# SGI-2022/Latent-Diffusion-Models-for-Shape-SDFs

Hardware: AMD Instinct MI355X
Metric: SDF queries/sec on 256^3 grid (+ DDPM sample steps/sec) (higher is better)
Workload: dtype bf16; 1 GPU; config4: decode B=64 shapes on a 256^3 grid on 1 rank (the whole grid is the one slab: no gather); batch=64, grid=256, latent_dim=256, decoder=DeepSDF 8x512 skip@4, parallelism=zslab1

## Files before the change

latent-diffusion-models-for-shape-sdfs_amd/csrc/decoder_common.h:

```cpp
#pragma once
#include "grid_index.h"
#include "ldm_internal.h"

#include <math.h>

namespace ldm {
namespace dec {

enum DecMode { kModeGrid = 0, kModePoints = 1, kModeBricks = 2 };

#define LDM_STR2(x) #x
#define LDM_STR(x) LDM_STR2(x)

__device__ __forceinline__ float grid_axis(int i, float vs, float origin) {
#pragma clang fp contract(off)
    float t = (float)i * vs;
    return t + origin;
}

__device__ __forceinline__ void grid_point(int p, int N, int k0, float vs, float origin,
                                           float& x, float& y, float& z) {
    const int nn = N * N;
    const int k = k0 + p / nn;
    const int r = p - (p / nn) * nn;
    const int j = r / N;
    const int i = r - j * N;
    x = grid_axis(i, vs, origin);
    y = grid_axis(j, vs, origin);
    z = grid_axis(k, vs, origin);
}


template <typename T>
struct Elem;
template <>
struct Elem<__bf16> {
    static __device__ __forceinline__ unsigned pack(float a, float b) {
        typedef float f32x2 __attribute__((ext_vector_type(2)));
        const f32x2 v = {a, b};
        return __builtin_bit_cast(unsigned, __builtin_convertvector(v, bf16x2));
    }
    static __device__ __forceinline__ float round(float x) { return (float)(__bf16)x; }
    static __device__ __forceinline__ f32x16 mfma(u32x4 a, u32x4 b, f32x16 c) {
        return __builtin_amdgcn_mfma_f32_32x32x16_bf16(__builtin_bit_cast(bf16x8, a),
                                                       __builtin_bit_cast(bf16x8, b), c, 0, 0, 0);
    }
    static __device__ __forceinline__ f32x16 mfma_v(u32x4 a, u32x4 b) {
        f32x16 d;
        asm volatile("v_mfma_f32_32x32x16_bf16 %0, %1, %2, 0" : "=&v"(d) : "v"(a), "v"(b));
        return d;
    }
    static __device__ __forceinline__ f32x4 mfma16(u32x4 a, u32x4 b, f32x4 c) {
        return __builtin_amdgcn_mfma_f32_16x16x32_bf16(__builtin_bit_cast(bf16x8, a),
                                                       __builtin_bit_cast(bf16x8, b), c, 0, 0, 0);
    }
};
template <>
struct Elem<_Float16> {
    static __device__ __forceinline__ unsigned pack(float a, float b) {
        f16x2 v = {(_Float16)a, (_Float16)b};
        return __builtin_bit_cast(unsigned, v);
    }
    static __device__ __forceinline__ float round(float x) { return (float)(_Float16)x; }
    static __device__ __forceinline__ f32x16 mfma(u32x4 a, u32x4 b, f32x16 c) {
        return __builtin_amdgcn_mfma_f32_32x32x16_f16(__builtin_bit_cast(f16x8, a),
                                                      __builtin_bit_cast(f16x8, b), c, 0, 0, 0);
    }
    static __device__ __forceinline__ f32x16 mfma_v(u32x4 a, u32x4 b) {
        f32x16 d;
        asm volatile("v_mfma_f32_32x32x16_f16 %0, %1, %2, 0" : "=&v"(d) : "v"(a), "v"(b));
        return d;
    }
    static __device__ __forceinline__ f32x4 mfma16(u32x4 a, u32x4 b, f32x4 c) {
        return __builtin_amdgcn_mfma_f32_16x16x32_f16(__builtin_bit_cast(f16x8, a),
                                                      __builtin_bit_cast(f16x8, b), c, 0, 0, 0);
    }
};


__device__ __forceinline__ unsigned relu2(unsigned v) {
    typedef short s16x2 __attribute__((ext_vector_type(2)));
    s16x2 x = __builtin_bit_cast(s16x2, v);
    const s16x2 z = {0, 0};
    x = __builtin_elementwise_max(x, z);
    return __builtin_bit_cast(unsigned, x);
}

template <typename T>
__device__ __forceinline__ void acc_to_frags(const f32x16& a, u32x4& f0, u32x4& f1) {
#pragma unroll
    for (int q = 0; q < 4; ++q) {
        f0[q] = relu2(Elem<T>::pack(a[2 * q], a[2 * q + 1]));
        f1[q] = relu2(Elem<T>::pack(a[8 + 2 * q], a[8 + 2 * q + 1]));
    }
}

}
}
```

latent-diffusion-models-for-shape-sdfs_amd/csrc/decoder_fs.hip:

```cpp
#include "decoder_common.h"

namespace ldm {
namespace {
using namespace dec;

constexpr int kFsD = 4;

constexpr int kFsStep = 2048;
constexpr int kFsAct = 33 * 4 * 1024;
constexpr int kFsRed = 4 * 4 * 64 * 4;
constexpr int kFsWl = 512 * 4;
#ifndef FS_STAMP
#define FS_STAMP 0
#endif
constexpr int kFsStamp = FS_STAMP ? 128 * 8 : 0;
#ifndef FS_ABL
#define FS_ABL 0
#endif
static_assert(FS_ABL == 0 || FS_STAMP, "ablations are diagnostic builds");
constexpr int kFsLds = kFsAct + kFsRed + kFsWl + kFsStamp;
static_assert(kFsLds <= 160 * 1024, "LDS");

__host__ __device__ constexpr int fs_nparts(int S) { return S == 256 ? 15 : 16; }
__host__ __device__ constexpr int fs_nsteps(int S) { return S == 256 ? 384 : 448; }

template <typename T>
__global__ void fs_aux_pack_kernel(const float* __restrict__ beta, const float* __restrict__ wxyz,
                                   int B, T* __restrict__ aux) {
    const int id = blockIdx.x * blockDim.x + threadIdx.x;
    if (id >= B * 4 * 4 * 2 * 64) return;
    const int lane = id & 63;
    const int i = (id >> 6) & 1;
    const int slot = (id >> 7) & 3;
    const int w = (id >> 9) & 3;
    const int b = id >> 11;
    const int li = slot >> 1;
    const int p = slot & 1;
    float v[8] = {0, 0, 0, 0, 0, 0, 0, 0};
    if (lane < 32) {
        const int f = 128 * w + 64 * p + 32 * i + lane;
        const float* wx = wxyz + ((size_t)li * kHidden + f) * 3;
        const float bb = beta[((size_t)b * 2 + li) * kHidden + f];
        const float hi = Elem<T>::round(bb);
        v[0] = wx[0]; v[1] = wx[1]; v[2] = wx[2];
        v[3] = wx[0]; v[4] = wx[1]; v[5] = wx[2];
        v[6] = hi;    v[7] = bb - hi;
    }
    T* o = aux + (size_t)id * 8;
#pragma unroll
    for (int e = 0; e < 8; ++e) o[e] = (T)v[e];
}

struct FArgs {
    const uint8_t* stream;
    const uint8_t* aux;
    const float* w_last;
    const float* xyz;
    float* out;
    float b_last;
    int npts, tiles_per_shape, n_tiles;
    int N, k0;
    float vs, origin;
    const int32_t* bricks;
    const int32_t* count;
    int nb, nbt;
    GridDiv gd;
};

enum FsEpi { FE_NONE = 0, FE_LATE = 1, FE_EARLY = 2, FE_FIN0 = 3, FE_FIN1 = 4, FE_CVT = 5,
             FE_WR = 6, FE_PIN = 8 };

struct FSrc {
    bool shape;
    uint32_t off;
    bool none = false;
};

struct FCtx {
    int lane, wave, h;
    uint32_t voff;
    char* smem;
    __amdgpu_buffer_rsrc_t rw;
    __amdgpu_buffer_rsrc_t ra;
    uint32_t s_beg, s_end;
    uint32_t s_iss;
    uint32_t baux_w;
    uint32_t aux_w;
    uint32_t aux_next;
    u32x4 auxn[2];
    u32x4 ring[kFsD][2];
    u32x4 b[4];
    float part[4];
    u32x4 ef[16];
    float* out;
    int npts, prev_shape, prev_local;
    float b_last;
    unsigned long long* st;
    int st_i;
    bool st_on;
    const int32_t* bricks;
    int N, nb, nbt;
};

__device__ __forceinline__ void stamp(FCtx& c) {
    if (FS_STAMP) {
        if (c.st_on && c.lane == 0 && c.st_i < 128) c.st[c.st_i] = __builtin_readcyclecounter();
        ++c.st_i;
    }
}

__device__ __forceinline__ u32x4 bld(__amdgpu_buffer_rsrc_t r, uint32_t voff, uint32_t soff) {
    return __builtin_bit_cast(u32x4, __builtin_amdgcn_raw_buffer_load_b128(r, voff, soff, 0));
}

__device__ __forceinline__ void load_aux(FCtx& c, FSrc s) {
    if (s.none) return;
    const __amdgpu_buffer_rsrc_t r = s.shape ? c.ra : c.rw;
    c.auxn[0] = bld(r, c.voff, s.off);
    c.auxn[1] = bld(r, c.voff + 1024u, s.off);
}

__device__ __forceinline__ uint32_t opaque(uint32_t v) {
    asm volatile("" : "+v"(v));
    return v;
}

__device__ __forceinline__ int opaque_s(int v) {
    asm volatile("" : "+s"(v));
    return v;
}

__device__ __forceinline__ char* lds_at(const FCtx& c, uint32_t off) {
    return c.smem + (opaque(c.voff) + off);
}
__device__ __forceinline__ u32x4* act_w(const FCtx& c, int late) {
    return reinterpret_cast<u32x4*>(lds_at(c, (uint32_t)(late + 4 * c.wave) * 4096u));
}
__device__ __forceinline__ const f32x4* wl_at(const FCtx& c, int p, int i) {
    const uint32_t h = opaque(c.voff) >> 9;
    return reinterpret_cast<const f32x4*>(
        c.smem + kFsAct + kFsRed + (((c.wave * 2 + p) * 2 + i) * 2) * 64 + h * 64);
}

__device__ __forceinline__ float* red_w(const FCtx& c) {
    return reinterpret_cast<float*>(c.smem + kFsAct + c.wave * 4 * 64 * 4 + (opaque(c.voff) >> 2));
}

__device__ __forceinline__ void fs_bar() {
    if (FS_ABL & 4) return;
    asm volatile("s_waitcnt lgkmcnt(0)\n\ts_barrier" ::: "memory");
}

__device__ __forceinline__ void read_b(FCtx& c, int pos) {
    const u32x4* p = reinterpret_cast<const u32x4*>(lds_at(c, pos * 4096));
#pragma unroll
    for (int n = 0; n < 4; ++n) c.b[n] = p[n * 64];
}

__device__ __forceinline__ void issue(FCtx& c, int r) {
    const uint32_t so = c.s_iss + (uint32_t)(r >> 1) * 2u * kFsStep;
    const uint32_t vo = c.voff + (uint32_t)(r & 1) * kFsStep;
    if (FS_ABL & 1) return;
    c.ring[r][0] = bld(c.rw, vo, so);
    c.ring[r][1] = bld(c.rw, vo + 1024u, so);
}

__device__ __forceinline__ void next_group(FCtx& c) {
    c.s_iss += 4u * kFsStep;
    if (c.s_iss == c.s_end) c.s_iss = c.s_beg;
}

__device__ __forceinline__ float relu_f(float x) {
    return __builtin_bit_cast(float, max(__builtin_bit_cast(int, x), 0));
}

__device__ __forceinline__ float acc_read(float a) {
    asm volatile("" : "+a"(a));
    return a;
}

template <typename T, int EKP>
__device__ __forceinline__ void epi_unit(FCtx& c, const f32x16 (&accY)[2][4], int u,
                                         u32x4* wbase) {
    constexpr int EK = EKP & 7;
    constexpr bool PIN = (EKP & FE_PIN) != 0 || EK == FE_FIN1;
    const int t = u >> 1, s = u & 1;
    const int i = t >> 2, n = t & 3;
    if (FS_ABL & 2) return;
    if (EK == FE_LATE || EK == FE_EARLY) {
        u32x4 f;
#pragma unroll
        for (int q = 0; q < 4; ++q) {
            const float lo = accY[i][n][8 * s + 2 * q], hi = accY[i][n][8 * s + 2 * q + 1];
            f[q] = relu2(PIN ? Elem<T>::pack(acc_read(lo), acc_read(hi)) : Elem<T>::pack(lo, hi));
        }
        wbase[((2 * i + s) * 4 + n) * 64] = f;
    } else if (EK == FE_FIN0 || EK == FE_FIN1) {
        const f32x4* w = wl_at(c, EK == FE_FIN0 ? 0 : 1, i);
        float part = c.part[n];
#pragma unroll
        for (int q = 2 * s; q < 2 * s + 2; ++q) {
            const f32x4 wv = w[q];
#pragma unroll
            for (int e = 0; e < 4; ++e) {
                const float v = PIN ? acc_read(accY[i][n][4 * q + e]) : accY[i][n][4 * q + e];
                part = fmaf(relu_f(v), wv[e], part);
            }
        }
        c.part[n] = part;
    }
}

template <typename T, int EKP>
__device__ __forceinline__ void epi_step(FCtx& c, const f32x16 (&accY)[2][4], int k,
                                         u32x4* wbase) {
    constexpr int EK = EKP & 7;
    if (EK == FE_NONE || k == 15) return;
    if (EK == FE_CVT) {
        if ((FS_ABL & 2) || k >= 8) return;
        u32x4 f0, f1;
#pragma unroll
        for (int q = 0; q < 4; ++q) {
            const f32x16& a = accY[k >> 2][k & 3];
            f0[q] = relu2(Elem<T>::pack(acc_read(a[2 * q]), acc_read(a[2 * q + 1])));
            f1[q] = relu2(Elem<T>::pack(acc_read(a[8 + 2 * q]), acc_read(a[8 + 2 * q + 1])));
        }
        c.ef[2 * k] = f0;
        c.ef[2 * k + 1] = f1;
        return;
    }
    if (EK == FE_WR) {
        if ((FS_ABL & 2) || k >= 4) return;
#pragma unroll
        for (int t = 2 * k; t < 2 * k + 2; ++t) {
            const int i = t >> 2, n = t & 3;
            wbase[(2 * i * 4 + n) * 64] = c.ef[2 * t];
            wbase[((2 * i + 1) * 4 + n) * 64] = c.ef[2 * t + 1];
        }
        return;
    }
    epi_unit<T, EKP>(c, accY, k, wbase);
    if (k == 14) epi_unit<T, EKP>(c, accY, 15, wbase);
    if (EK == FE_FIN0 && k == 14) {
#pragma unroll
        for (int n = 0; n < 4; ++n) asm volatile("" : "+v"(c.part[n]));
    }
    if (EK == FE_FIN1 && k == 14) {
        float* rw = red_w(c);
#pragma unroll
        for (int n = 0; n < 4; ++n) {
            rw[n * 64] = c.part[n];
            c.part[n] = 0.f;
        }
    }
}

__device__ __forceinline__ void fin_store(const FCtx& c, int shape, int local) {
    const int lane = (int)(opaque(c.voff) >> 4);
    if (local < 0 || lane >= 32) return;
    const float* rr = reinterpret_cast<const float*>(
        c.smem + kFsAct + c.wave * 64 * 4 + (opaque(c.voff) >> 2));
    float s = 0.f;
#pragma unroll
    for (int w = 0; w < 4; ++w) s += rr[w * 4 * 64] + rr[w * 4 * 64 + 32];
    const int pt = local * kTilePoints + 32 * c.wave + lane;
    if (pt < c.npts) {
        const __amdgpu_buffer_rsrc_t ro = __builtin_amdgcn_make_buffer_rsrc(
            (void*)(c.out + (size_t)shape * c.npts), (short)0, 0x7ffffff0, 0x00020000);
        __builtin_amdgcn_raw_buffer_store_b32(__builtin_bit_cast(uint32_t, tanhf(s + c.b_last)),
                                              ro, (uint32_t)pt * 4u, 0, 2 );
    }
}

__device__ __forceinline__ int list_at(const int32_t* list, int i) {
    typedef const __attribute__((address_space(4))) int32_t* const_i32;
    return ((const_i32)(uintptr_t)list)[i];
}

__device__ __forceinline__ void brick_origin(int gid, int nb_, int& shape, int& i0, int& j0,
                                             int& k0) {
    const int nb = opaque_s(nb_);
    const int nb2 = nb * nb, nb3 = nb2 * nb;
    shape = gid / nb3;
    const int id = gid - shape * nb3;
    const int bz = id / nb2, r = id - bz * nb2;
    const int by = r / nb;
    i0 = 8 * (r - by * nb);
    j0 = 8 * by;
    k0 = 8 * bz;
}

__device__ __forceinline__ void fin_store_bricks(const FCtx& c, int tile) {
    const int lane = (int)(opaque(c.voff) >> 4);
    if (tile < 0 || lane >= 32) return;
    const float* rr = reinterpret_cast<const float*>(
        c.smem + kFsAct + c.wave * 64 * 4 + (opaque(c.voff) >> 2));
    float s = 0.f;
#pragma unroll
    for (int w = 0; w < 4; ++w) s += rr[w * 4 * 64] + rr[w * 4 * 64 + 32];
    const int gid = list_at(c.bricks, tile >> 2);
    LDM_DASSERT(gid >= 0 && gid < c.nbt);
    int shape, i0, j0, k0;
    brick_origin(gid, c.nb, shape, i0, j0, k0);
    const int idx = 128 * (tile & 3) + 32 * c.wave + lane;
    const int i = i0 + (idx & 7), j = j0 + ((idx >> 3) & 7);
    const int k = k0 + 2 * (tile & 3) + (c.wave >> 1);
    const int N = c.N;
    if ((unsigned)gid < (unsigned)c.nbt && i < N && j < N && k < N) {
        const __amdgpu_buffer_rsrc_t ro = __builtin_amdgcn_make_buffer_rsrc(
            (void*)(c.out + ((size_t)shape * N + k) * N * N), (short)0, 0x7ffffff0, 0x00020000);
        __builtin_amdgcn_raw_buffer_store_b32(__builtin_bit_cast(uint32_t, tanhf(s + c.b_last)),
                                              ro, (uint32_t)(j * N + i) * 4u, 0, 2 );
    }
}

template <int MODE>
__device__ __forceinline__ void fin_store_mode(const FCtx& c) {
    if (MODE == kModeBricks) fin_store_bricks(c, c.prev_local);
    else fin_store(c, c.prev_shape, c.prev_local);
}

__device__ __forceinline__ void valu_slot(int v) {
    if (v == 2) __builtin_amdgcn_sched_group_barrier(0x002, 2, 0);
    else if (v == 4) __builtin_amdgcn_sched_group_barrier(0x002, 4, 0);
}

template <typename T>
__device__ __forceinline__ void mfma_pair(f32x16 (&acc)[2][4], const u32x4& a0, const u32x4& a1,
                                          const u32x4& b, int n) {
    acc[0][n] = Elem<T>::mfma(a0, b, acc[0][n]);
    acc[1][n] = Elem<T>::mfma(a1, b, acc[1][n]);
}

template <typename T, int EKP, int K0, int BAR>
__device__ __forceinline__ void group4(FCtx& c, f32x16 (&acc)[2][4], const f32x16 (&accY)[2][4],
                                       int p0) {
    constexpr int EK = EKP & 7;
    constexpr int BP = 1;
    u32x4* wbase = nullptr;
    if (EK == FE_LATE) wbase = act_w(c, 16);
    if (EK == FE_EARLY || EK == FE_WR) wbase = act_w(c, 0);
    const char* gbase = lds_at(c, (p0 + 1) * 4096);
#pragma unroll
    for (int r = 0; r < 4; ++r) {
        const u32x4* nb = reinterpret_cast<const u32x4*>(gbase + r * 4096);
        const u32x4 a0 = c.ring[r][0], a1 = c.ring[r][1];
        const int k = K0 + r;
        const int V = (EK == FE_NONE || EK == FE_WR || k == 15) ? 0
                      : (k == 14 || EK == FE_CVT) ? 4 : 2;
        if (r == BAR) {
#pragma unroll
            for (int n = 0; n < BP; ++n) mfma_pair<T>(acc, a0, a1, c.b[n], n);
            for (int n = 0; n < BP; ++n) {
                __builtin_amdgcn_sched_group_barrier(0x008, 2, 0);
            }
            __builtin_amdgcn_sched_barrier(0);
            fs_bar();
            __builtin_amdgcn_sched_barrier(0);
#pragma unroll
            for (int n = 0; n < BP; ++n) c.b[n] = nb[n * 64];
#pragma unroll
            for (int n = BP; n < 4; ++n) {
                mfma_pair<T>(acc, a0, a1, c.b[n], n);
                c.b[n] = nb[n * 64];
            }
            issue(c, r);
            epi_step<T, EKP>(c, accY, k, wbase);
            for (int n = 0; n < BP; ++n) __builtin_amdgcn_sched_group_barrier(0x100, 1, 0);
            for (int n = BP; n < 4; ++n) {
                __builtin_amdgcn_sched_group_barrier(0x008, 1, 0);
                valu_slot(V);
                __builtin_amdgcn_sched_group_barrier(0x008, 1, 0);
                __builtin_amdgcn_sched_group_barrier(0x100, 1, 0);
                valu_slot(V);
            }
        } else {
#pragma unroll
            for (int n = 0; n < 4; ++n) {
                mfma_pair<T>(acc, a0, a1, c.b[n], n);
                c.b[n] = nb[n * 64];
            }
            issue(c, r);
            epi_step<T, EKP>(c, accY, k, wbase);
#pragma unroll
            for (int n = 0; n < 4; ++n) {
                __builtin_amdgcn_sched_group_barrier(0x008, 1, 0);
                valu_slot(V);
                __builtin_amdgcn_sched_group_barrier(0x008, 1, 0);
                __builtin_amdgcn_sched_group_barrier(0x100, 1, 0);
                valu_slot(V);
            }
        }
        __builtin_amdgcn_sched_group_barrier(0x020, 2, 0);
        __builtin_amdgcn_sched_barrier(0);
    }
    next_group(c);
}

template <typename T, int EK, bool BAR>
__device__ __forceinline__ void steps16e(FCtx& c, f32x16 (&acc)[2][4],
                                         const f32x16 (&accY)[2][4], int p0) {
    group4<T, EK, 0, -1>(c, acc, accY, p0);
    group4<T, EK, 4, -1>(c, acc, accY, p0 + 4);
    group4<T, EK, 8, -1>(c, acc, accY, p0 + 8);
    group4<T, EK, 12, BAR ? 3 : -1>(c, acc, accY, p0 + 12);
}

template <typename T>
__device__ __forceinline__ void steps_plain(FCtx& c, f32x16 (&acc)[2][4],
                                            const f32x16 (&accY)[2][4], int pos0, int j0, int j1) {
#pragma unroll 1
    for (int j = j0; j < j1; j += 4) group4<T, FE_NONE, 0, -1>(c, acc, accY, pos0 + j);
}

template <typename T, int EKP, bool E16, int MODE = kModeGrid>
__device__ __forceinline__ void run_part(FCtx& c, f32x16 (&acc)[2][4], const f32x16 (&accY)[2][4],
                                         int nk, bool mid, bool endbar, FSrc naux, int pos0,
                                         bool bar0) {
    constexpr int EK = EKP & 7;
    const f32x16 zero = {};
    const u32x4 a0 = c.auxn[0], a1 = c.auxn[1];
    if (bar0) {
#pragma unroll
        for (int n = 0; n < 4; ++n) {
            acc[0][n] = Elem<T>::mfma(a0, c.b[n], zero);
            acc[1][n] = Elem<T>::mfma(a1, c.b[n], zero);
        }
        load_aux(c, naux);
        fs_bar();
        read_b(c, pos0);
    } else {
        const u32x4* p = reinterpret_cast<const u32x4*>(lds_at(c, pos0 * 4096));
#pragma unroll
        for (int n = 0; n < 4; ++n) {
            acc[0][n] = Elem<T>::mfma(a0, c.b[n], zero);
            acc[1][n] = Elem<T>::mfma(a1, c.b[n], zero);
            c.b[n] = p[n * 64];
        }
        load_aux(c, naux);
#pragma unroll
        for (int n = 0; n < 4; ++n) {
            __builtin_amdgcn_sched_group_barrier(0x008, 2, 0);
            __builtin_amdgcn_sched_group_barrier(0x100, 1, 0);
        }
        __builtin_amdgcn_sched_group_barrier(0x020, 2, 0);
        __builtin_amdgcn_sched_barrier(0);
    }
    if (EK == FE_NONE) {
#pragma unroll
        for (int i = 0; i < 2; ++i)
#pragma unroll
            for (int n = 0; n < 4; ++n) asm volatile("" ::"a"(accY[i][n]));
    }
    stamp(c);
    if (!E16 && EK != FE_NONE) {
        if (mid || (endbar && nk == 16)) steps16e<T, EKP, true>(c, acc, accY, pos0);
        else steps16e<T, EKP, false>(c, acc, accY, pos0);
        if (EK == FE_FIN1) {
            stamp(c);
            fin_store_mode<MODE>(c);
        }
        stamp(c);
        if (endbar && nk == 32) {
            steps_plain<T>(c, acc, accY, pos0, 16, 28);
            group4<T, FE_NONE, 0, 3>(c, acc, accY, pos0 + 28);
        } else {
            steps_plain<T>(c, acc, accY, pos0, 16, nk);
        }
    } else if (E16 && (EKP & FE_PIN)) {
        steps_plain<T>(c, acc, accY, pos0, 0, 12);
        group4<T, FE_NONE, 0, 3>(c, acc, accY, pos0 + 12);
        stamp(c);
        if (endbar) steps16e<T, EKP, true>(c, acc, accY, pos0 + 16);
        else steps16e<T, EKP, false>(c, acc, accY, pos0 + 16);
    } else if (E16) {
        static_assert(!E16 || EK == FE_EARLY, "E16 parts convert part 0 of their own layer");
        steps_plain<T>(c, acc, accY, pos0, 0, 8);
        group4<T, FE_CVT, 0, -1>(c, acc, accY, pos0 + 8);
        group4<T, FE_CVT, 4, 3>(c, acc, accY, pos0 + 12);
        stamp(c);
        group4<T, FE_WR, 0, -1>(c, acc, accY, pos0 + 16);
        steps_plain<T>(c, acc, accY, pos0, 20, 28);
        group4<T, FE_NONE, 0, 3>(c, acc, accY, pos0 + 28);
    } else {
        steps_plain<T>(c, acc, accY, pos0, 0, nk < 16 ? nk : 16);
        stamp(c);
        steps_plain<T>(c, acc, accY, pos0, 16, nk);
    }
    stamp(c);
}

template <typename T>
__device__ __forceinline__ void acc_to_lds(FCtx& c, const f32x16 (&acc)[2][4]) {
    u32x4* p = act_w(c, 16);
#pragma unroll
    for (int i = 0; i < 2; ++i)
#pragma unroll
        for (int n = 0; n < 4; ++n) {
            u32x4 f0, f1;
            acc_to_frags<T>(acc[i][n], f0, f1);
            p[(2 * i * 4 + n) * 64] = f0;
            p[((2 * i + 1) * 4 + n) * 64] = f1;
        }
}

template <typename T, bool LATE>
__device__ __forceinline__ void layer0_part(FCtx& c, FSrc naux) {
    const u32x4 a[2] = {c.auxn[0], c.auxn[1]};
    u32x4* p = act_w(c, LATE ? 16 : 0);
    f32x16 t[2];
    t[0] = Elem<T>::mfma_v(a[0], c.b[0]);
#pragma unroll
    for (int q = 0; q < 8; ++q) {
        const int i = q & 1, n = q >> 1;
        if (q < 7) t[(q + 1) & 1] = Elem<T>::mfma_v(a[(q + 1) & 1], c.b[(q + 1) >> 1]);
        if (q == 0) {
            asm volatile("s_nop 10" : "+v"(t[0]));
            load_aux(c, naux);
            stamp(c);
        }
        __builtin_amdgcn_sched_barrier(0);
        u32x4 f0, f1;
        acc_to_frags<T>(t[q & 1], f0, f1);
        p[(2 * i * 4 + n) * 64] = f0;
        p[((2 * i + 1) * 4 + n) * 64] = f1;
        __builtin_amdgcn_sched_barrier(0);
    }
    stamp(c);
}

template <typename T, int S, int MODE>
__global__ __launch_bounds__(256, 1) void dec_fs_kernel(FArgs a) {
    __shared__ __attribute__((aligned(16))) char smem[kFsLds];
    FCtx c;
    c.lane = threadIdx.x & 63;
    c.wave = __builtin_amdgcn_readfirstlane(threadIdx.x >> 6);
// ... 74 lines not shown
        stamp(c);
        load_aux(c, shp(0));
        const uint32_t lv = opaque(c.voff);
        const bool hi = lv >= 512u;
        const uint32_t p0 = (uint32_t)local * kTilePoints;
        uint32_t ti = 0, tj = 0, tk = 0;
        if (MODE == kModeGrid) {
            grid_first(p0, (uint32_t)a.N, a.gd, ti, tj, tk);
            tk += (uint32_t)a.k0;
        }
        const float* row = nullptr;
        if (MODE == kModePoints) {
            row = a.xyz + (size_t)shape * a.npts * 3;
            asm volatile("" : "+s"(row));
        }
#pragma unroll
        for (int n = 0; n < 4; ++n) {
            int pt = local * kTilePoints + 32 * n + (int)((lv >> 4) & 31u);
            if (pt >= a.npts) pt = a.npts - 1;
            float x, y, z;
            if (MODE == kModeBricks) {
                const int idx = 128 * (tile & 3) + 32 * n + (int)((lv >> 4) & 31u);
                const int m = a.N - 1;
                x = grid_axis(min(bi0 + (idx & 7), m), a.vs, a.origin);
                y = grid_axis(min(bj0 + ((idx >> 3) & 7), m), a.vs, a.origin);
                z = grid_axis(min(bk0 + (idx >> 6), m), a.vs, a.origin);
            } else if (MODE == kModePoints) {
                const float* qq = row + (size_t)pt * 3;
                x = qq[0];
                y = qq[1];
                z = qq[2];
            } else {
                const uint32_t off =
                    grid_tail_off(p0, 32u * n + ((lv >> 4) & 31u), (uint32_t)a.npts);
                uint32_t vi, vj, vk;
                grid_voxel(ti, tj, tk, off, (uint32_t)a.N, a.gd.m, vi, vj, vk);
                x = grid_axis((int)vi, a.vs, a.origin);
                y = grid_axis((int)vj, a.vs, a.origin);
                z = grid_axis((int)vk, a.vs, a.origin);
            }
            const float xh = Elem<T>::round(x), yh = Elem<T>::round(y), zh = Elem<T>::round(z);
            u32x4 f;
            f[0] = hi ? 0u : Elem<T>::pack(xh, yh);
            f[1] = hi ? 0u : Elem<T>::pack(zh, x - xh);
            f[2] = hi ? 0u : Elem<T>::pack(y - yh, z - zh);
            f[3] = hi ? 0u : Elem<T>::pack(1.f, 1.f);
            reinterpret_cast<u32x4*>(lds_at(c, 32u * 4096u))[n * 64] = f;
        }
        read_b(c, 32);

        layer0_part<T, false>(c, shp(1));
        layer0_part<T, true>(c, bias(2));

        constexpr int kPinW = S == 512 ? FE_PIN : 0;
        int pi = 2;
        run_part<T, FE_FIN1, false, MODE>(c, accA, accB, 32, true, false, bias(pi + 1), 0, true);
        run_part<T, FE_EARLY, true>(c, accB, accA, 32, true, true, bias(pi + 2), 0, false);
        pi += 2;
        constexpr int L2P = S == 256 ? 3 : 4;
#pragma unroll 1
        for (int l = 2; l < L2P; ++l, pi += 2) {
            const FSrc nx = (S == 512 && l == 3) ? shp(2) : bias(pi + 2);
            run_part<T, FE_LATE | kPinW, false>(c, accA, accB, 32, true, false, bias(pi + 1), 0,
                                                false);
            run_part<T, FE_EARLY | FE_PIN, true>(c, accB, accA, 32, true, true, nx, 0, false);
        }
        if (S == 256) {
            run_part<T, FE_LATE | kPinW, false>(c, accA, accB, 32, true, false, shp(2), 0,
                                                false);
            fs_bar();
            acc_to_lds<T>(c, accA);
            stamp(c);
            run_part<T, FE_NONE, false>(c, accA, accB, 16, false, false, shp(3), 16, true);
            run_part<T, FE_EARLY | FE_PIN, false>(c, accB, accA, 16, false, true, bias(pi + 3),
                                                  16, false);
            pi += 3;
        } else {
            run_part<T, FE_LATE | kPinW, false>(c, accA, accB, 32, true, false, shp(3), 0,
                                                false);
            run_part<T, FE_EARLY | FE_PIN, true>(c, accB, accA, 32, true, true, bias(pi + 2), 0,
                                                 false);
            pi += 2;
        }
#pragma unroll 1
        for (int l = 5; l < 7; ++l, pi += 2) {
            run_part<T, FE_LATE | FE_PIN, false>(c, accA, accB, 32, true, false, bias(pi + 1), 0,
                                                 false);
            run_part<T, FE_EARLY | FE_PIN, true>(c, accB, accA, 32, true, true, bias(pi + 2), 0,
                                                 false);
        }
        run_part<T, FE_LATE | FE_PIN, false>(c, accA, accB, 32, true, false, bias(pi + 1), 0,
                                             false);
        run_part<T, FE_FIN0 | FE_PIN, false>(c, accB, accA, 32, false, true, FSrc{true, 0, true},
                                             0, false);
        c.prev_shape = shape;
        c.prev_local = local;
        c.aux_w = c.aux_next;
    }
#pragma unroll
    for (int u = 0; u < 16; ++u) epi_unit<T, FE_FIN1>(c, accB, u, nullptr);
    {
        float* rw = red_w(c);
#pragma unroll
        for (int n = 0; n < 4; ++n) rw[n * 64] = c.part[n];
    }
    fs_bar();
    fin_store_mode<MODE>(c);
    asm volatile("s_waitcnt vmcnt(0)" ::: "memory");
    if (FS_STAMP && c.wave == 0) {
        __builtin_amdgcn_s_waitcnt(0);
        for (int k = c.lane; k < 128; k += 64)
            reinterpret_cast<unsigned long long*>(a.out)[(size_t)blockIdx.x * 128 + k] = c.st[k];
    }
}

template <typename T, int S>
void launch_fs(const FArgs& a, bool points, hipStream_t s, int grid) {
    if (points)
        hipLaunchKernelGGL((dec_fs_kernel<T, S, kModePoints>), dim3(grid), dim3(256), 0, s, a);
    else
        hipLaunchKernelGGL((dec_fs_kernel<T, S, kModeGrid>), dim3(grid), dim3(256), 0, s, a);
}

template <typename T, int S>
void launch_fs_bricks(const FArgs& a, hipStream_t s, int grid) {
    hipLaunchKernelGGL((dec_fs_kernel<T, S, kModeBricks>), dim3(grid), dim3(256), 0, s, a);
}

}

size_t decoder_fs_aux_bytes(int B) { return (size_t)B * 4 * 4 * kFsStep; }

int decoder_fs_n_stages(int skip_width) { return fs_nsteps(skip_width == 253 ? 256 : 512); }

int decoder_fs_fwd(const ldm_decoder_t* w, const float* beta, const float* xyz, int B, int npts,
                   int N, int k0, float vs, float origin, float* out, void* ws, size_t ws_bytes,
                   hipStream_t s, int num_cus, const int32_t* bricks, const int32_t* count,
                   int n_bricks) {
    const int S = w->skip_width == 253 ? 256 : 512;
    LDM_REQUIRE(w->n_stages == fs_nsteps(S), LDM_EINVAL, "split layout: n_stages %d != %d",
                w->n_stages, fs_nsteps(S));
    LDM_REQUIRE(ws != nullptr && ws_bytes >= decoder_fs_aux_bytes(B) && LDM_ALIGNED(ws, 16),
                LDM_ENOSPC, "workspace too small: need %zu bytes, got %zu",
                decoder_fs_aux_bytes(B), ws_bytes);
    LDM_REQUIRE((size_t)B * 4 * 4 * kFsStep < 0x7ffffff0u, LDM_EINVAL,
                "split layout: %d shapes exceed the aux buffer range", B);
    {
        const int n = B * 4 * 4 * 2 * 64;
        if (w->dtype == LDM_BF16)
            hipLaunchKernelGGL(fs_aux_pack_kernel<__bf16>, dim3((n + 255) / 256), dim3(256), 0, s,
                               beta, w->wxyz, B, (__bf16*)ws);
        else
            hipLaunchKernelGGL(fs_aux_pack_kernel<_Float16>, dim3((n + 255) / 256), dim3(256), 0,
// ... 46 lines not shown
```

Measured before the change: 457.7 million queries/s.

## Interleave accumulator epilogue with MFMA pairs via inline asm windows

Replaces the separate epilogue step (epi_unit/epi_step with FE_PIN/FE_CVT/FE_WR variants) with hand-scheduled inline-asm MFMA pairs. Each pair reads previous-layer accumulators from AGPRs, converts and applies relu, or accumulates the final-layer dot product, in the shadow of the matrix ops. It also precomputes LDS base pointers per 16-step group and carries the stream issue offset across groups, which cuts address arithmetic. The aim is to hide VALU epilogue work behind MFMA latency, but the fixed asm ordering limits what the compiler can schedule and adds register-pressure risk.

```diff
diff --git a/latent-diffusion-models-for-shape-sdfs_amd/csrc/decoder_common.h b/latent-diffusion-models-for-shape-sdfs_amd/csrc/decoder_common.h
--- a/latent-diffusion-models-for-shape-sdfs_amd/csrc/decoder_common.h
+++ b/latent-diffusion-models-for-shape-sdfs_amd/csrc/decoder_common.h
@@ -31,6 +31,120 @@
 }
 
 
+#define LDM_PAIR_OPS(MFMA, CVT)                                                                   \
+                                                                       \
+    template <bool TAIL>                                                                          \
+    static __device__ __forceinline__ void pair_cvt1(f32x16& c0, f32x16& c1, const u32x4& a0,     \
+                                                     const u32x4& a1, const u32x4& b, float e0,   \
+                                                     float e1, unsigned& w) {                     \
+        unsigned t0, t1;                                                                          \
+        if (!TAIL)                                                                                \
+            asm volatile(MFMA " %0, %5, %7, %0\n\t"                                               \
+                         "v_accvgpr_read_b32 %3, %8\n\t"                                          \
+                         "v_accvgpr_read_b32 %4, %9\n\t"                                          \
+                         MFMA " %1, %6, %7, %1\n\t"                                               \
+                         CVT " %2, %3, %4\n\t"                                                    \
+                         "v_pk_max_i16 %2, %2, 0"                                                 \
+                         : "+a"(c0), "+a"(c1), "=&v"(w), "=&v"(t0), "=&v"(t1)                     \
+                         : "v"(a0), "v"(a1), "v"(b), "a"(e0), "a"(e1));                           \
+        else                                                                                      \
+            asm volatile(MFMA " %0, %5, %7, %0\n\t"                                               \
+                         "v_accvgpr_read_b32 %3, %8\n\t"                                          \
+                         "v_accvgpr_read_b32 %4, %9\n\t"                                          \
+                         CVT " %2, %3, %4\n\t"                                                    \
+                         "v_pk_max_i16 %2, %2, 0\n\t"                                             \
+                         MFMA " %1, %6, %7, %1"                                                   \
+                         : "+a"(c0), "+a"(c1), "=&v"(w), "=&v"(t0), "=&v"(t1)                     \
+                         : "v"(a0), "v"(a1), "v"(b), "a"(e0), "a"(e1));                           \
+    }                                                                                             \
+                                                                                  \
+    template <bool TAIL>                                                                          \
+    static __device__ __forceinline__ void pair_cvt2(f32x16& c0, f32x16& c1, const u32x4& a0,     \
+                                                     const u32x4& a1, const u32x4& b, float e0,   \
+                                                     float e1, float e2, float e3, unsigned& w0,  \
+                                                     unsigned& w1) {                              \
+        unsigned t0, t1;                                                                          \
+        if (!TAIL)                                                                                \
+            asm volatile(MFMA " %0, %6, %8, %0\n\t"                                               \
+                         "v_accvgpr_read_b32 %4, %9\n\t"                                          \
+                         "v_accvgpr_read_b32 %5, %10\n\t"                                         \
+                         CVT " %2, %4, %5\n\t"                                                    \
+                         "v_pk_max_i16 %2, %2, 0\n\t"                                             \
+                         MFMA " %1, %7, %8, %1\n\t"                                               \
+                         "v_accvgpr_read_b32 %4, %11\n\t"                                         \
+                         "v_accvgpr_read_b32 %5, %12\n\t"                                         \
+                         CVT " %3, %4, %5\n\t"                                                    \
+                         "v_pk_max_i16 %3, %3, 0"                                                 \
+                         : "+a"(c0), "+a"(c1), "=&v"(w0), "=&v"(w1), "=&v"(t0), "=&v"(t1)         \
+                         : "v"(a0), "v"(a1), "v"(b), "a"(e0), "a"(e1), "a"(e2), "a"(e3));         \
+        else                                                                                      \
+            asm volatile(MFMA " %0, %6, %8, %0\n\t"                                               \
+                         "v_accvgpr_read_b32 %4, %9\n\t"                                          \
+                         "v_accvgpr_read_b32 %5, %10\n\t"                                         \
+                         CVT " %2, %4, %5\n\t"                                                    \
+                         "v_pk_max_i16 %2, %2, 0\n\t"                                             \
+                         "v_accvgpr_read_b32 %4, %11\n\t"                                         \
+                         "v_accvgpr_read_b32 %5, %12\n\t"                                         \
+                         MFMA " %1, %7, %8, %1\n\t"                                               \
+                         CVT " %3, %4, %5\n\t"                                                    \
+                         "v_pk_max_i16 %3, %3, 0"                                                 \
+                         : "+a"(c0), "+a"(c1), "=&v"(w0), "=&v"(w1), "=&v"(t0), "=&v"(t1)         \
+                         : "v"(a0), "v"(a1), "v"(b), "a"(e0), "a"(e1), "a"(e2), "a"(e3));         \
+    }                                                                                             \
+              \
+    template <bool TAIL>                                                                          \
+    static __device__ __forceinline__ void pair_fin(f32x16& c0, f32x16& c1, const u32x4& a0,      \
+                                                    const u32x4& a1, const u32x4& b, float e0,    \
+                                                    float e1, float w0, float w1, float& p) {     \
+        float t0, t1;                                                                             \
+        if (!TAIL)                                                                                \
+            asm volatile(MFMA " %0, %5, %7, %0\n\t"                                               \
+                         "v_accvgpr_read_b32 %3, %8\n\t"                                          \
+                         "v_accvgpr_read_b32 %4, %9\n\t"                                          \
+                         "v_max_i32_e32 %3, 0, %3\n\t"                                            \
+                         "v_max_i32_e32 %4, 0, %4\n\t"                                            \
+                         MFMA " %1, %6, %7, %1\n\t"                                               \
+                         "v_fmac_f32_e32 %2, %3, %10\n\t"                                         \
+                         "v_fmac_f32_e32 %2, %4, %11"                                             \
+                         : "+a"(c0), "+a"(c1), "+v"(p), "=&v"(t0), "=&v"(t1)                      \
+                         : "v"(a0), "v"(a1), "v"(b), "a"(e0), "a"(e1), "v"(w0), "v"(w1));         \
+        else                                                                                      \
+            asm volatile(MFMA " %0, %5, %7, %0\n\t"                                               \
+                         "v_accvgpr_read_b32 %3, %8\n\t"                                          \
+                         "v_accvgpr_read_b32 %4, %9\n\t"                                          \
+                         "v_max_i32_e32 %3, 0, %3\n\t"                                            \
+                         "v_max_i32_e32 %4, 0, %4\n\t"                                            \
+                         "v_fmac_f32_e32 %2, %3, %10\n\t"                                         \
+                         "v_fmac_f32_e32 %2, %4, %11\n\t"                                         \
+                         MFMA " %1, %6, %7, %1"                                                   \
+                         : "+a"(c0), "+a"(c1), "+v"(p), "=&v"(t0), "=&v"(t1)                      \
+                         : "v"(a0), "v"(a1), "v"(b), "a"(e0), "a"(e1), "v"(w0), "v"(w1));         \
+    }                                                                                             \
+                    \
+    static __device__ __forceinline__ void pair_fin3(f32x16& c0, f32x16& c1, const u32x4& a0,     \
+                                                     const u32x4& a1, const u32x4& b, float e0,   \
+                                                     float e1, float w0, float w1, float& p,      \
+                                                     float x, float wx, float& q) {               \
+        float t0, t1, t2;                                                                         \
+        asm volatile(MFMA " %0, %7, %9, %0\n\t"                                                   \
+                     "v_accvgpr_read_b32 %4, %10\n\t"                                             \
+                     "v_accvgpr_read_b32 %5, %11\n\t"                                             \
+                     "v_max_i32_e32 %4, 0, %4\n\t"                                                \
+                     "v_max_i32_e32 %5, 0, %5\n\t"                                                \
+                     "v_accvgpr_read_b32 %6, %12\n\t"                                             \
+                     MFMA " %1, %8, %9, %1\n\t"                                                   \
+                     "v_fmac_f32_e32 %2, %4, %13\n\t"                                             \
+                     "v_fmac_f32_e32 %2, %5, %14\n\t"                                             \
+                     "v_max_i32_e32 %6, 0, %6\n\t"                                                \
+                     "v_fmac_f32_e32 %3, %6, %15"                                                 \
+                     : "+a"(c0), "+a"(c1), "+v"(p), "+v"(q), "=&v"(t0), "=&v"(t1), "=&v"(t2)      \
+                     : "v"(a0), "v"(a1), "v"(b), "a"(e0), "a"(e1), "a"(x), "v"(w0), "v"(w1),      \
+                       "v"(wx));                                                                  \
+    }
+
+#define LDM_CVT_BF16 "v_cvt_pk_bf16_f32"
+#define LDM_CVT_F16 "v_cvt_pk_f16_f32"
+
 template <typename T>
 struct Elem;
 template <>
@@ -54,6 +168,7 @@
         return __builtin_amdgcn_mfma_f32_16x16x32_bf16(__builtin_bit_cast(bf16x8, a),
                                                        __builtin_bit_cast(bf16x8, b), c, 0, 0, 0);
     }
+    LDM_PAIR_OPS("v_mfma_f32_32x32x16_bf16", LDM_CVT_BF16)
 };
 template <>
 struct Elem<_Float16> {
@@ -75,6 +190,7 @@
         return __builtin_amdgcn_mfma_f32_16x16x32_f16(__builtin_bit_cast(f16x8, a),
                                                       __builtin_bit_cast(f16x8, b), c, 0, 0, 0);
     }
+    LDM_PAIR_OPS("v_mfma_f32_32x32x16_f16", LDM_CVT_F16)
 };
 
 
diff --git a/latent-diffusion-models-for-shape-sdfs_amd/csrc/decoder_fs.hip b/latent-diffusion-models-for-shape-sdfs_amd/csrc/decoder_fs.hip
--- a/latent-diffusion-models-for-shape-sdfs_amd/csrc/decoder_fs.hip
+++ b/latent-diffusion-models-for-shape-sdfs_amd/csrc/decoder_fs.hip
@@ -67,8 +67,7 @@
     GridDiv gd;
 };
 
-enum FsEpi { FE_NONE = 0, FE_LATE = 1, FE_EARLY = 2, FE_FIN0 = 3, FE_FIN1 = 4, FE_CVT = 5,
-             FE_WR = 6, FE_PIN = 8 };
+enum FsEpi { FE_NONE = 0, FE_LATE = 1, FE_EARLY = 2, FE_FIN0 = 3, FE_FIN1 = 4 };
 
 struct FSrc {
     bool shape;
@@ -91,7 +90,8 @@
     u32x4 ring[kFsD][2];
     u32x4 b[4];
     float part[4];
-    u32x4 ef[16];
+    const f32x4* wlp;
+    f32x4 wl[2][4];
     float* out;
     int npts, prev_shape, prev_local;
     float b_last;
@@ -133,6 +133,12 @@
 __device__ __forceinline__ char* lds_at(const FCtx& c, uint32_t off) {
     return c.smem + (opaque(c.voff) + off);
 }
+__device__ __forceinline__ char* lds_base(const FCtx& c, uint32_t off) {
+    return c.smem + opaque(opaque(c.voff) + off);
+}
+__device__ __forceinline__ u32x4* act_wb(const FCtx& c, int late) {
+    return reinterpret_cast<u32x4*>(lds_base(c, (uint32_t)(late + 4 * c.wave) * 4096u));
+}
 __device__ __forceinline__ u32x4* act_w(const FCtx& c, int late) {
     return reinterpret_cast<u32x4*>(lds_at(c, (uint32_t)(late + 4 * c.wave) * 4096u));
 }
@@ -165,10 +171,11 @@
     c.ring[r][1] = bld(c.rw, vo + 1024u, so);
 }
 
-__device__ __forceinline__ void next_group(FCtx& c) {
-    c.s_iss += 4u * kFsStep;
-    if (c.s_iss == c.s_end) c.s_iss = c.s_beg;
-}
+__device__ __forceinline__ uint32_t next_iss(const FCtx& c) {
+    const uint32_t n = c.s_iss + 4u * kFsStep;
+    return n == c.s_end ? c.s_beg : n;
+}
+__device__ __forceinline__ void next_group(FCtx& c) { c.s_iss = next_iss(c); }
 
 __device__ __forceinline__ float relu_f(float x) {
     return __builtin_bit_cast(float, max(__builtin_bit_cast(int, x), 0));
@@ -179,80 +186,141 @@
     return a;
 }
 
-template <typename T, int EKP>
-__device__ __forceinline__ void epi_unit(FCtx& c, const f32x16 (&accY)[2][4], int u,
-                                         u32x4* wbase) {
-    constexpr int EK = EKP & 7;
-    constexpr bool PIN = (EKP & FE_PIN) != 0 || EK == FE_FIN1;
+__device__ __forceinline__ void fin1_unit(FCtx& c, const f32x16 (&accY)[2][4], int u) {
     const int t = u >> 1, s = u & 1;
     const int i = t >> 2, n = t & 3;
-    if (FS_ABL & 2) return;
-    if (EK == FE_LATE || EK == FE_EARLY) {
+    const f32x4* w = wl_at(c, 1, i);
+    float part = c.part[n];
+#pragma unroll
+    for (int q = 2 * s; q < 2 * s + 2; ++q) {
+        const f32x4 wv = w[q];
+#pragma unroll
+        for (int e = 0; e < 4; ++e)
+            part = fmaf(relu_f(acc_read(accY[i][n][4 * q + e])), wv[e], part);
+    }
+    c.part[n] = part;
+}
+
+template <typename T>
+__device__ __forceinline__ void mfma_pair(f32x16 (&acc)[2][4], const u32x4& a0, const u32x4& a1,
+                                          const u32x4& b, int n) {
+    acc[0][n] = Elem<T>::mfma(a0, b, acc[0][n]);
+    acc[1][n] = Elem<T>::mfma(a1, b, acc[1][n]);
+}
+
+template <typename T>
+__device__ __forceinline__ void window_step(FCtx& c, f32x16 (&acc)[2][4],
+                                            const f32x16 (&accY)[2][4], const u32x4& a0,
+                                            const u32x4& a1, const u32x4* nb, int k, int r,
+                                            u32x4* wbase) {
+    uint32_t nxt = 0;
+    if (k < 14) {
+        const int t = k >> 1, s = k & 1;
+        const int i = t >> 2, nn = t & 3;
         u32x4 f;
 #pragma unroll
-        for (int q = 0; q < 4; ++q) {
-            const float lo = accY[i][n][8 * s + 2 * q], hi = accY[i][n][8 * s + 2 * q + 1];
-            f[q] = relu2(PIN ? Elem<T>::pack(acc_read(lo), acc_read(hi)) : Elem<T>::pack(lo, hi));
-        }
-        wbase[((2 * i + s) * 4 + n) * 64] = f;
-    } else if (EK == FE_FIN0 || EK == FE_FIN1) {
-        const f32x4* w = wl_at(c, EK == FE_FIN0 ? 0 : 1, i);
-        float part = c.part[n];
-#pragma unroll
-        for (int q = 2 * s; q < 2 * s + 2; ++q) {
-            const f32x4 wv = w[q];
-#pragma unroll
-            for (int e = 0; e < 4; ++e) {
-                const float v = PIN ? acc_read(accY[i][n][4 * q + e]) : accY[i][n][4 * q + e];
-                part = fmaf(relu_f(v), wv[e], part);
+        for (int n = 0; n < 4; ++n) {
+            unsigned w;
+            if (r == 3 && n == 1) nxt = next_iss(c);
+            const float e0 = accY[i][nn][8 * s + 2 * n], e1 = accY[i][nn][8 * s + 2 * n + 1];
+            if (n < 3)
+                Elem<T>::template pair_cvt1<false>(acc[0][n], acc[1][n], a0, a1, c.b[n], e0, e1,
+                                                   w);
+            else
+                Elem<T>::template pair_cvt1<true>(acc[0][n], acc[1][n], a0, a1, c.b[n], e0, e1,
+                                                  w);
+            f[n] = w;
+            c.b[n] = nb[n * 64];
+            __builtin_amdgcn_sched_barrier(0);
+        }
+        issue(c, r);
+        wbase[((2 * i + s) * 4 + nn) * 64] = f;
+        if (r == 3) c.s_iss = nxt;
+    } else {
+        u32x4 f[2];
+        const f32x16& y = accY[1][3];
+#pragma unroll
+        for (int p = 0; p < 4; ++p) {
+            unsigned w0, w1;
+            if (p < 3)
+                Elem<T>::template pair_cvt2<false>(acc[0][p], acc[1][p], a0, a1, c.b[p], y[4 * p],
+                                                   y[4 * p + 1], y[4 * p + 2], y[4 * p + 3], w0,
+                                                   w1);
+            else
+                Elem<T>::template pair_cvt2<true>(acc[0][p], acc[1][p], a0, a1, c.b[p], y[4 * p],
+                                                  y[4 * p + 1], y[4 * p + 2], y[4 * p + 3], w0,
+                                                  w1);
+            f[p >> 1][2 * (p & 1)] = w0;
+            f[p >> 1][2 * (p & 1) + 1] = w1;
+            c.b[p] = nb[p * 64];
+            if (p == 1) wbase[(2 * 4 + 3) * 64] = f[0];
+            __builtin_amdgcn_sched_barrier(0);
+        }
+        issue(c, r);
+        wbase[(3 * 4 + 3) * 64] = f[1];
+    }
+    __builtin_amdgcn_sched_barrier(0);
+}
+
+template <typename T, int P>
+__device__ __forceinline__ void window_step_fin(FCtx& c, f32x16 (&acc)[2][4],
+                                                const f32x16 (&accY)[2][4], const u32x4& a0,
+                                                const u32x4& a1, const u32x4* nb, int k, int r) {
+    const int t = k >> 1, s = k & 1;
+    const int i = t >> 2, nn = t & 3;
+    const f32x16& y = accY[1][3];
+    uint32_t nxt = 0;
+    if (k == 0) {
+        c.wlp = wl_at(c, P, 0);
+#pragma unroll
+        for (int q = 0; q < 4; ++q) c.wl[0][q] = c.wlp[q];
+    }
+#pragma unroll
+    for (int n = 0; n < 4; ++n) {
+        if (k < 14) {
+            const int e = 8 * s + 2 * n;
+            const float e0 = accY[i][nn][e], e1 = accY[i][nn][e + 1];
+            const float w0 = c.wl[i][e >> 2][e & 3], w1 = c.wl[i][e >> 2][(e & 3) + 1];
+            const int x = 2 * (k - 8) + n;
+            if (k >= 8 && n < 2)
+                Elem<T>::pair_fin3(acc[0][n], acc[1][n], a0, a1, c.b[n], e0, e1, w0, w1,
+                                   c.part[nn], y[x], c.wl[1][x >> 2][x & 3], c.part[3]);
+            else if (n < 3)
+                Elem<T>::template pair_fin<false>(acc[0][n], acc[1][n], a0, a1, c.b[n], e0, e1,
+                                                  w0, w1, c.part[nn]);
+            else
+                Elem<T>::template pair_fin<true>(acc[0][n], acc[1][n], a0, a1, c.b[n], e0, e1,
+                                                 w0, w1, c.part[nn]);
+        } else if (n < 2) {
+            const int x = 12 + 2 * n;
+            Elem<T>::template pair_fin<false>(acc[0][n], acc[1][n], a0, a1, c.b[n], y[x],
+                                              y[x + 1], c.wl[1][3][x & 3],
+                                              c.wl[1][3][(x & 3) + 1],
+                                              c.part[3]);
+        } else {
+            mfma_pair<T>(acc, a0, a1, c.b[n], n);
+        }
+        if (r == 3 && n == 2) nxt = next_iss(c);
+        c.b[n] = nb[n * 64];
+        if (k == 6) c.wl[1][n] = c.wlp[8 + n];
+        if (k == 14 && n == 2) {
+            if (P == 0) {
+#pragma unroll
+                for (int m = 0; m < 4; ++m) asm volatile("" : "+v"(c.part[m]));
+            } else {
+                float* rw = red_w(c);
+#pragma unroll
+                for (int m = 0; m < 4; ++m) {
+                    rw[m * 64] = c.part[m];
+                    c.part[m] = 0.f;
+                }
             }
         }
-        c.part[n] = part;
-    }
-}
-
-template <typename T, int EKP>
-__device__ __forceinline__ void epi_step(FCtx& c, const f32x16 (&accY)[2][4], int k,
-                                         u32x4* wbase) {
-    constexpr int EK = EKP & 7;
-    if (EK == FE_NONE || k == 15) return;
-    if (EK == FE_CVT) {
-        if ((FS_ABL & 2) || k >= 8) return;
-        u32x4 f0, f1;
-#pragma unroll
-        for (int q = 0; q < 4; ++q) {
-            const f32x16& a = accY[k >> 2][k & 3];
-            f0[q] = relu2(Elem<T>::pack(acc_read(a[2 * q]), acc_read(a[2 * q + 1])));
-            f1[q] = relu2(Elem<T>::pack(acc_read(a[8 + 2 * q]), acc_read(a[8 + 2 * q + 1])));
-        }
-        c.ef[2 * k] = f0;
-        c.ef[2 * k + 1] = f1;
-        return;
-    }
-    if (EK == FE_WR) {
-        if ((FS_ABL & 2) || k >= 4) return;
-#pragma unroll
-        for (int t = 2 * k; t < 2 * k + 2; ++t) {
-            const int i = t >> 2, n = t & 3;
-            wbase[(2 * i * 4 + n) * 64] = c.ef[2 * t];
-            wbase[((2 * i + 1) * 4 + n) * 64] = c.ef[2 * t + 1];
-        }
-        return;
-    }
-    epi_unit<T, EKP>(c, accY, k, wbase);
-    if (k == 14) epi_unit<T, EKP>(c, accY, 15, wbase);
-    if (EK == FE_FIN0 && k == 14) {
-#pragma unroll
-        for (int n = 0; n < 4; ++n) asm volatile("" : "+v"(c.part[n]));
-    }
-    if (EK == FE_FIN1 && k == 14) {
-        float* rw = red_w(c);
-#pragma unroll
-        for (int n = 0; n < 4; ++n) {
-            rw[n * 64] = c.part[n];
-            c.part[n] = 0.f;
-        }
-    }
+        __builtin_amdgcn_sched_barrier(0);
+    }
+    issue(c, r);
+    if (r == 3) c.s_iss = nxt;
+    __builtin_amdgcn_sched_barrier(0);
 }
 
 __device__ __forceinline__ void fin_store(const FCtx& c, int shape, int local) {
@@ -320,34 +388,26 @@
     else fin_store(c, c.prev_shape, c.prev_local);
 }
 
-__device__ __forceinline__ void valu_slot(int v) {
-    if (v == 2) __builtin_amdgcn_sched_group_barrier(0x002, 2, 0);
-    else if (v == 4) __builtin_amdgcn_sched_group_barrier(0x002, 4, 0);
-}
-
-template <typename T>
-__device__ __forceinline__ void mfma_pair(f32x16 (&acc)[2][4], const u32x4& a0, const u32x4& a1,
-                                          const u32x4& b, int n) {
-    acc[0][n] = Elem<T>::mfma(a0, b, acc[0][n]);
-    acc[1][n] = Elem<T>::mfma(a1, b, acc[1][n]);
-}
-
-template <typename T, int EKP, int K0, int BAR>
+template <typename T, int EK, int K0, int BAR, bool WIN = false>
 __device__ __forceinline__ void group4(FCtx& c, f32x16 (&acc)[2][4], const f32x16 (&accY)[2][4],
-                                       int p0) {
-    constexpr int EK = EKP & 7;
+                                       int p0, const char* gb = nullptr, u32x4* wb = nullptr,
+                                       uint32_t* go = nullptr) {
+    static_assert(WIN || EK == FE_NONE, "windows run through steps16e");
     constexpr int BP = 1;
-    u32x4* wbase = nullptr;
-    if (EK == FE_LATE) wbase = act_w(c, 16);
-    if (EK == FE_EARLY || EK == FE_WR) wbase = act_w(c, 0);
-    const char* gbase = lds_at(c, (p0 + 1) * 4096);
+    const bool carry = go != nullptr;
+    const char* gbase = WIN ? gb : carry ? c.smem + *go + 4096 : lds_base(c, (p0 + 1) * 4096);
 #pragma unroll
     for (int r = 0; r < 4; ++r) {
-        const u32x4* nb = reinterpret_cast<const u32x4*>(gbase + r * 4096);
+        const bool last = carry && r == 3;
+        uint32_t nxt = 0;
+        if (last) {
+            nxt = next_iss(c);
+            *go = opaque(*go + 4u * 4096u);
+        }
+        const u32x4* nb =
+            reinterpret_cast<const u32x4*>(last ? c.smem + *go : gbase + r * 4096);
         const u32x4 a0 = c.ring[r][0], a1 = c.ring[r][1];
         const int k = K0 + r;
-        const int V = (EK == FE_NONE || EK == FE_WR || k == 15) ? 0
-                      : (k == 14 || EK == FE_CVT) ? 4 : 2;
         if (r == BAR) {
 #pragma unroll
             for (int n = 0; n < BP; ++n) mfma_pair<T>(acc, a0, a1, c.b[n], n);
@@ -365,15 +425,19 @@
                 c.b[n] = nb[n * 64];
             }
             issue(c, r);
-            epi_step<T, EKP>(c, accY, k, wbase);
             for (int n = 0; n < BP; ++n) __builtin_amdgcn_sched_group_barrier(0x100, 1, 0);
             for (int n = BP; n < 4; ++n) {
-                __builtin_amdgcn_sched_group_barrier(0x008, 1, 0);
-                valu_slot(V);
-                __builtin_amdgcn_sched_group_barrier(0x008, 1, 0);
+                __builtin_amdgcn_sched_group_barrier(0x008, 2, 0);
                 __builtin_amdgcn_sched_group_barrier(0x100, 1, 0);
-                valu_slot(V);
             }
+        } else if ((EK == FE_LATE || EK == FE_EARLY) && k < 15 && !(FS_ABL & 2)) {
+            window_step<T>(c, acc, accY, a0, a1, nb, k, r, wb);
+            if (r == 3) return;
+            continue;
+        } else if ((EK == FE_FIN0 || EK == FE_FIN1) && k < 15 && !(FS_ABL & 2)) {
+            window_step_fin<T, EK == FE_FIN1>(c, acc, accY, a0, a1, nb, k, r);
+            if (r == 3) return;
+            continue;
         } else {
 #pragma unroll
             for (int n = 0; n < 4; ++n) {
@@ -381,43 +445,48 @@
                 c.b[n] = nb[n * 64];
             }
             issue(c, r);
-            epi_step<T, EKP>(c, accY, k, wbase);
+            if (last) c.s_iss = nxt;
 #pragma unroll
             for (int n = 0; n < 4; ++n) {
-                __builtin_amdgcn_sched_group_barrier(0x008, 1, 0);
-                valu_slot(V);
-                __builtin_amdgcn_sched_group_barrier(0x008, 1, 0);
+                __builtin_amdgcn_sched_group_barrier(0x008, 2, 0);
+                if (last && n == 0) {
+                    __builtin_amdgcn_sched_group_barrier(0x004, 3, 0);
+                    __builtin_amdgcn_sched_group_barrier(0x002, 1, 0);
+                }
                 __builtin_amdgcn_sched_group_barrier(0x100, 1, 0);
-                valu_slot(V);
             }
         }
         __builtin_amdgcn_sched_group_barrier(0x020, 2, 0);
         __builtin_amdgcn_sched_barrier(0);
     }
-    next_group(c);
+    if (!carry) next_group(c);
 }
 
 template <typename T, int EK, bool BAR>
 __device__ __forceinline__ void steps16e(FCtx& c, f32x16 (&acc)[2][4],
                                          const f32x16 (&accY)[2][4], int p0) {
-    group4<T, EK, 0, -1>(c, acc, accY, p0);
-    group4<T, EK, 4, -1>(c, acc, accY, p0 + 4);
-    group4<T, EK, 8, -1>(c, acc, accY, p0 + 8);
-    group4<T, EK, 12, BAR ? 3 : -1>(c, acc, accY, p0 + 12);
+    const char* gb = lds_base(c, (p0 + 1) * 4096);
+    u32x4* wb = EK == FE_LATE ? act_wb(c, 16) : EK == FE_EARLY ? act_wb(c, 0) : nullptr;
+    group4<T, EK, 0, -1, true>(c, acc, accY, p0, gb, wb);
+    group4<T, EK, 4, -1, true>(c, acc, accY, p0 + 4, gb + 4 * 4096, wb);
+    group4<T, EK, 8, -1, true>(c, acc, accY, p0 + 8, gb + 8 * 4096, wb);
+    group4<T, EK, 12, BAR ? 3 : -1, true>(c, acc, accY, p0 + 12, gb + 12 * 4096, wb);
 }
 
 template <typename T>
 __device__ __forceinline__ void steps_plain(FCtx& c, f32x16 (&acc)[2][4],
                                             const f32x16 (&accY)[2][4], int pos0, int j0, int j1) {
+    if (j0 >= j1) return;
+    uint32_t go = opaque(opaque(c.voff) + (uint32_t)(pos0 + j0) * 4096u);
 #pragma unroll 1
-    for (int j = j0; j < j1; j += 4) group4<T, FE_NONE, 0, -1>(c, acc, accY, pos0 + j);
-}
-
-template <typename T, int EKP, bool E16, int MODE = kModeGrid>
+    for (int j = j0; j < j1; j += 4)
+        group4<T, FE_NONE, 0, -1>(c, acc, accY, pos0 + j, nullptr, nullptr, &go);
+}
+
+template <typename T, int EK, bool E16, int MODE = kModeGrid>
 __device__ __forceinline__ void run_part(FCtx& c, f32x16 (&acc)[2][4], const f32x16 (&accY)[2][4],
                                          int nk, bool mid, bool endbar, FSrc naux, int pos0,
                                          bool bar0) {
-    constexpr int EK = EKP & 7;
     const f32x16 zero = {};
     const u32x4 a0 = c.auxn[0], a1 = c.auxn[1];
     if (bar0) {
@@ -454,8 +523,8 @@
     }
     stamp(c);
     if (!E16 && EK != FE_NONE) {
-        if (mid || (endbar && nk == 16)) steps16e<T, EKP, true>(c, acc, accY, pos0);
-        else steps16e<T, EKP, false>(c, acc, accY, pos0);
+        if (mid || (endbar && nk == 16)) steps16e<T, EK, true>(c, acc, accY, pos0);
+        else steps16e<T, EK, false>(c, acc, accY, pos0);
         if (EK == FE_FIN1) {
             stamp(c);
             fin_store_mode<MODE>(c);
@@ -467,21 +536,13 @@
         } else {
             steps_plain<T>(c, acc, accY, pos0, 16, nk);
         }
-    } else if (E16 && (EKP & FE_PIN)) {
+    } else if (E16) {
+        static_assert(!E16 || EK == FE_EARLY, "E16 parts convert part 0 of their own layer");
         steps_plain<T>(c, acc, accY, pos0, 0, 12);
         group4<T, FE_NONE, 0, 3>(c, acc, accY, pos0 + 12);
         stamp(c);
-        if (endbar) steps16e<T, EKP, true>(c, acc, accY, pos0 + 16);
-        else steps16e<T, EKP, false>(c, acc, accY, pos0 + 16);
-    } else if (E16) {
-        static_assert(!E16 || EK == FE_EARLY, "E16 parts convert part 0 of their own layer");
-        steps_plain<T>(c, acc, accY, pos0, 0, 8);
-        group4<T, FE_CVT, 0, -1>(c, acc, accY, pos0 + 8);
-        group4<T, FE_CVT, 4, 3>(c, acc, accY, pos0 + 12);
-        stamp(c);
-        group4<T, FE_WR, 0, -1>(c, acc, accY, pos0 + 16);
-        steps_plain<T>(c, acc, accY, pos0, 20, 28);
-        group4<T, FE_NONE, 0, 3>(c, acc, accY, pos0 + 28);
+        if (endbar) steps16e<T, EK, true>(c, acc, accY, pos0 + 16);
+        else steps16e<T, EK, false>(c, acc, accY, pos0 + 16);
     } else {
         steps_plain<T>(c, acc, accY, pos0, 0, nk < 16 ? nk : 16);
         stamp(c);
@@ -662,7 +723,6 @@
         layer0_part<T, false>(c, shp(1));
         layer0_part<T, true>(c, bias(2));
 
-        constexpr int kPinW = S == 512 ? FE_PIN : 0;
         int pi = 2;
         run_part<T, FE_FIN1, false, MODE>(c, accA, accB, 32, true, false, bias(pi + 1), 0, true);
         run_part<T, FE_EARLY, true>(c, accB, accA, 32, true, true, bias(pi + 2), 0, false);
@@ -671,44 +731,44 @@
 #pragma unroll 1
         for (int l = 2; l < L2P; ++l, pi += 2) {
             const FSrc nx = (S == 512 && l == 3) ? shp(2) : bias(pi + 2);
-            run_part<T, FE_LATE | kPinW, false>(c, accA, accB, 32, true, false, bias(pi + 1), 0,
+            run_part<T, FE_LATE, false>(c, accA, accB, 32, true, false, bias(pi + 1), 0,
                                                 false);
-            run_part<T, FE_EARLY | FE_PIN, true>(c, accB, accA, 32, true, true, nx, 0, false);
+            run_part<T, FE_EARLY, true>(c, accB, accA, 32, true, true, nx, 0, false);
         }
         if (S == 256) {
-            run_part<T, FE_LATE | kPinW, false>(c, accA, accB, 32, true, false, shp(2), 0,
+            run_part<T, FE_LATE, false>(c, accA, accB, 32, true, false, shp(2), 0,
                                                 false);
             fs_bar();
             acc_to_lds<T>(c, accA);
             stamp(c);
             run_part<T, FE_NONE, false>(c, accA, accB, 16, false, false, shp(3), 16, true);
-            run_part<T, FE_EARLY | FE_PIN, false>(c, accB, accA, 16, false, true, bias(pi + 3),
+            run_part<T, FE_EARLY, false>(c, accB, accA, 16, false, true, bias(pi + 3),
                                                   16, false);
             pi += 3;
         } else {
-            run_part<T, FE_LATE | kPinW, false>(c, accA, accB, 32, true, false, shp(3), 0,
+            run_part<T, FE_LATE, false>(c, accA, accB, 32, true, false, shp(3), 0,
                                                 false);
-            run_part<T, FE_EARLY | FE_PIN, true>(c, accB, accA, 32, true, true, bias(pi + 2), 0,
+            run_part<T, FE_EARLY, true>(c, accB, accA, 32, true, true, bias(pi + 2), 0,
                                                  false);
             pi += 2;
         }
 #pragma unroll 1
         for (int l = 5; l < 7; ++l, pi += 2) {
-            run_part<T, FE_LATE | FE_PIN, false>(c, accA, accB, 32, true, false, bias(pi + 1), 0,
+            run_part<T, FE_LATE, false>(c, accA, accB, 32, true, false, bias(pi + 1), 0,
                                                  false);
-            run_part<T, FE_EARLY | FE_PIN, true>(c, accB, accA, 32, true, true, bias(pi + 2), 0,
+            run_part<T, FE_EARLY, true>(c, accB, accA, 32, true, true, bias(pi + 2), 0,
                                                  false);
         }
-        run_part<T, FE_LATE | FE_PIN, false>(c, accA, accB, 32, true, false, bias(pi + 1), 0,
+        run_part<T, FE_LATE, false>(c, accA, accB, 32, true, false, bias(pi + 1), 0,
                                              false);
-        run_part<T, FE_FIN0 | FE_PIN, false>(c, accB, accA, 32, false, true, FSrc{true, 0, true},
+        run_part<T, FE_FIN0, false>(c, accB, accA, 32, false, true, FSrc{true, 0, true},
                                              0, false);
         c.prev_shape = shape;
         c.prev_local = local;
         c.aux_w = c.aux_next;
     }
 #pragma unroll
-    for (int u = 0; u < 16; ++u) epi_unit<T, FE_FIN1>(c, accB, u, nullptr);
+    for (int u = 0; u < 16; ++u) fin1_unit(c, accB, u);
     {
         float* rw = red_w(c);
 #pragma unroll
```

Result: faster. 473.9 million queries/s, median of 6 (+3.5%).
